# ignaschuemer7/soft-actor-critic

Hardware: AMD Instinct MI355X
Metric: SAC gradient steps/sec + replay-sample GB/s, BipedalWalker batch=256 (higher is better)
Workload: dtype fp32; 1 GPU; c2: BipedalWalker-v3 obs=24 act=4 2x[256, 256] MLPs, buffer=1000000, batch=256, auto-alpha, device sampler, fp32 arithmetic; global_batch=256, parallelism=replicas1, graph_chunk=64

## Files before the change

### soft-actor-critic_amd/csrc/sac_phases.h

```cpp
#pragma once
#include <type_traits>
#include <utility>

#include "sac_device.h"
#include "sac_math.h"

#define SAC_DEV_LAYERS 6

__device__ __forceinline__ __amdgpu_buffer_rsrc_t coh_rsrc(const void* base, uint32_t bytes) {
  return __builtin_amdgcn_make_buffer_rsrc((void*)base, (short)0, (int)bytes, 0x00020000);
}
template <bool COH>
__device__ __forceinline__ void coh_store16(const void* base, uint32_t byte_off, u32x4 v) {
  __builtin_amdgcn_raw_buffer_store_b128(__builtin_bit_cast(__attribute__((ext_vector_type(4))) unsigned, v),
                                         coh_rsrc(base, 0xFFFFFFF0u), (int)byte_off, 0, COH ? 16 : 0);
}
__device__ __forceinline__ float coh_load(const float* p) {
  return __hip_atomic_load((float*)p, __ATOMIC_RELAXED, __HIP_MEMORY_SCOPE_AGENT);
}
template <bool COH>
__device__ __forceinline__ float ldf(const float* p) {
  if constexpr (COH) return coh_load(p);
  return *GPC(float, p);
}
// ... 304 lines not shown
      constexpr int u = decltype(uc)::value;
      f0[u] = coh_frag<T, COH>(rs, o0 + u * FSB);
      f1[u] = coh_frag<T, COH>(rs, o1 + u * FSB);
    });
  }
  F a[NCH][RT];
  static_for<NCH>([&](auto uc) {
    constexpr int u = decltype(uc)::value;
#pragma unroll
    for (int rt = 0; rt < RT; ++rt) a[u][rt] = MM<T>::from_lds(arow + rt * 16 * lda + u * KC);
  });
  f32x4 acc0[RT], acc1[RT];
#pragma unroll
  for (int rt = 0; rt < RT; ++rt) acc0[rt] = acc1[rt] = (f32x4){0.f, 0.f, 0.f, 0.f};
  static_for<NCH>([&](auto uc) {
    constexpr int u = decltype(uc)::value;
#pragma unroll
    for (int rt = 0; rt < RT; ++rt) {
      MM<T>::mma(acc0[rt], a[u][rt], f0[u]);
      MM<T>::mma(acc1[rt], a[u][rt], f1[u]);
    }
  });
  epi(0, nt0 * 16 + c, acc0, true);
  epi(1, nt1 * 16 + c, acc1, true);
}

template <typename T, int ROWS, int HC, typename Epi>
__device__ __forceinline__ void gemm_step(const lf* __restrict__ A, int lda, const GemmW& w, Epi epi,
                                          const Held<T, HC ? HC : 1>* held) {
  constexpr int RT = ROWS / 16;
  constexpr int KC = MM<T>::KC, KL = MM<T>::KL;
  const int lane = threadIdx.x & 63, wave = wave_id();
  const int c = lane & 15, g = lane >> 4;
  const int NT = w.NT, nch = w.cols / KC;
  const lf* arow = A + c * lda + g * KL;
  if (w.NT == 2 * SAC_NW) {
    if (nch == 8) {
      gemm_pair_fixed<T, RT, 8, false, HC>(arow, lda, w, lane, wave, c, epi, held);
      return;
    }
    if (nch == 1) {
      gemm_pair_fixed<T, RT, 1, false, HC>(arow, lda, w, lane, wave, c, epi, held);
      return;
    }
  }
  const __amdgpu_buffer_rsrc_t rs = coh_rsrc(w.p, 0xFFFFFFF0u);
  auto pair = [&](int nt0, bool first) __attribute__((always_inline)) {
    const int nt1 = nt0 + SAC_NW;
    const bool has1 = nt1 < NT;
    const uint32_t o0 = (uint32_t)(packed_lane<T>(nt0, w.tcols, lane) * sizeof(T));
    const uint32_t o1 = (uint32_t)(packed_lane<T>(has1 ? nt1 : nt0, w.tcols, lane) * sizeof(T));
    f32x4 acc0[RT], acc1[RT];
#pragma unroll
    for (int rt = 0; rt < RT; ++rt) acc0[rt] = acc1[rt] = (f32x4){0.f, 0.f, 0.f, 0.f};
    if (HC > 0 && first && held && held->tag == w.p) {
      const int hn = nch < HC ? nch : HC;
      if (hn == HC) {
        mma_batch<T, RT, (HC ? HC : 1)>(arow, lda, 0, has1, held->f0, held->f1, acc0, acc1);
      } else {
        static_for<(HC ? HC : 1)>([&](auto uc) {
          constexpr int u = decltype(uc)::value;
          if (u < hn)
#pragma unroll
            for (int rt = 0; rt < RT; ++rt) {
              const typename MM<T>::Frag a = MM<T>::from_lds(arow + rt * 16 * lda + u * KC);
              MM<T>::mma(acc0[rt], a, held->f0[u]);
              if (has1) MM<T>::mma(acc1[rt], a, held->f1[u]);
            }
        });
      }
      if (hn < nch) mma_pair_from<T, RT, 8>(arow, lda, rs, o0, o1, has1, hn, nch, acc0, acc1);
    } else {
      mma_pair_from<T, RT, 8>(arow, lda, rs, o0, o1, has1, 0, nch, acc0, acc1);
    }
    epi(0, nt0 * 16 + c, acc0, first);
    if (has1) epi(1, nt1 * 16 + c, acc1, first);
  };
  bool first = true;
  for (int nt0 = wave; nt0 < NT; nt0 += 2 * SAC_NW) {
    pair(nt0, first);
    first = false;
  }
}

template <int ROWS>
__device__ __forceinline__ void act_pass_fwd(lf* Y, int ldy, int NT, int act) {
  const int lane = threadIdx.x & 63, wave = wave_id();
  const int c = lane & 15, g = lane >> 4;
#pragma unroll 1
  for (int nt = wave; nt < NT; nt += SAC_NW)
#pragma unroll 1
    for (int e = 0; e < ROWS / 4; ++e) {
      const int r = (e >> 2) * 16 + g * 4 + (e & 3);
      lf* y = Y + r * ldy + nt * 16 + c;
      *y = act_fwd(act, *y);
    }
}
template <int ROWS>
__device__ __forceinline__ void act_pass_bwd(lf* G, int ldg, const lf* P, int ldp, int NT, int K, int act) {
  const int lane = threadIdx.x & 63, wave = wave_id();
  const int c = lane & 15, g = lane >> 4;
#pragma unroll 1
  for (int nt = wave; nt < NT; nt += SAC_NW) {
    const int k = nt * 16 + c;
    if (k >= K) continue;
#pragma unroll 1
    for (int e = 0; e < ROWS / 4; ++e) {
      const int r = (e >> 2) * 16 + g * 4 + (e & 3);
      G[r * ldg + k] = act_bwd(act, P[r * ldp + k], G[r * ldg + k]);
    }
  }
}

template <typename T, int ROWS, int HC = 0>
__device__ __forceinline__ void layer_fwd(const lf* X, int ldx, const AS_C LayerDev& L, const float* bias_, int act, lf* P,
                                          int ldp, lf* Y, int ldy, float* Pg_, int pg_row0,
                                          const Held<T, HC ? HC : 1>* held = nullptr) {
  const AS_G float* bias = GPC(float, bias_);
  AS_G float* Pg = GP(float, Pg_);
  const int lane = threadIdx.x & 63, wave = wave_id();
  const int g = lane >> 4;
  const int N = L.N, Np = L.Np;
  const int n0 = wave * 16 + (lane & 15), n1 = n0 + 16 * SAC_NW;
  const GemmW w = gw_fwd(L);
  const bool hb = HC > 0 && held && held->tag == w.p;
  const float bpre0 = hb ? held->b0 : ldf<false>((const float*)bias + (n0 < N ? n0 : N - 1));
  const float bpre1 = hb ? held->b1 : ldf<false>((const float*)bias + (n1 < N ? n1 : N - 1));
  gemm_step<T, ROWS, HC>(X, ldx, w, [&](int h, int n, const f32x4* acc, bool first) {
    const bool nv = n < N;
    const float bn = first ? (h ? bpre1 : bpre0) : ldf<false>((const float*)bias + (nv ? n : N - 1));
#pragma unroll
    for (int rt = 0; rt < ROWS / 16; ++rt)
#pragma unroll
      for (int i = 0; i < 4; ++i) {
        const int r = rt * 16 + g * 4 + i;
        const float p = nv ? acc[rt][i] + bn : 0.f;
        if (P) P[r * ldp + n] = p;
        Y[r * ldy + n] = act == ACT_RELU ? (p > 0.f ? p : 0.f) : p;
        if (Pg && r >= pg_row0) Pg[(size_t)(r - pg_row0) * Np + n] = p;
      }
  }, held);
  if (act != ACT_RELU && act != ACT_ID) act_pass_fwd<ROWS>(Y, ldy, Np >> 4, act);
}

template <typename T, int ROWS, int HC = 0>
__device__ __forceinline__ void layer_bwd(const lf* G, int ldg, const AS_C LayerDev& L, const lf* Pprev, int ldp,
                                          int act_prev, lf* Gout, int ldo, const Held<T, HC ? HC : 1>* held = nullptr) {
  const int g = (threadIdx.x & 63) >> 4;
  const int K = L.K;
  gemm_step<T, ROWS, HC>(G, ldg, gw_bwd(L), [&](int, int k, const f32x4* acc, bool) {
    const bool kv = k < K;
#pragma unroll
    for (int rt = 0; rt < ROWS / 16; ++rt)
#pragma unroll
      for (int i = 0; i < 4; ++i) {
        const int r = rt * 16 + g * 4 + i;
        float v = kv ? acc[rt][i] : 0.f;
        if (act_prev == ACT_RELU && !(Pprev[r * ldp + k] > 0.f)) v = 0.f;
        Gout[r * ldo + k] = v;
      }
  }, held);
  if (act_prev >= 0 && act_prev != ACT_RELU && act_prev != ACT_ID)
    act_pass_bwd<ROWS>(Gout, ldo, Pprev, ldp, L.Kp >> 4, K, act_prev);
}

template <typename T, int ROWS>
__device__ __forceinline__ void store_T(const lf* __restrict__ src, int lds_ld, int Kp, int K, void* dst_,
                                                 int Bp, int col0, int nvalid, float* dbp_,
                                                 const lf* __restrict__ rowscale = nullptr, int dbp_ld = 0) {
  AS_G T* dst = GP(T, dst_);
  AS_G float* dbp = GP(float, dbp_);
  constexpr int CH = ROWS / 8;
  const int span = (Kp * CH + 63) / 64 * 64;
  for (int i = threadIdx.x; i < span; i += SAC_THREADS) {
    const bool live = i < Kp * CH;
    const int k = i / CH, ch = i % CH;
    T v[8];
    float s = 0.f, xv[8];
#pragma unroll
    for (int q = 0; q < 8; ++q) xv[q] = src[(ch * 8 + q) * lds_ld + (live ? k : 0)];
    if (rowscale) {
      float sc[8];
#pragma unroll
      for (int q = 0; q < 8; ++q) sc[q] = rowscale[ch * 8 + q];
#pragma unroll
      for (int q = 0; q < 8; ++q) xv[q] = sc[q] * xv[q];
    }
#pragma unroll
    for (int q = 0; q < 8; ++q) {
      const int r = ch * 8 + q;
      const float x = (live && r < nvalid && k < K) ? xv[q] : 0.f;
      s += x;
      v[q] = MM<T>::cvt(x);
    }
    if (live) {
      AS_G T* d = dst + (size_t)k * Bp + col0 + ch * 8;
      if constexpr (sizeof(T) == 2) {
        *(AS_G u32x4*)d = *(const u32x4*)v;
      } else {
        *(AS_G u32x4*)d = *(const u32x4*)v;
        *(AS_G u32x4*)(d + 4) = *(const u32x4*)(v + 4);
      }
    }
    if (dbp) {
#pragma unroll
      for (int o = 1; o < CH; o <<= 1) s += __shfl_xor(s, o, 64);
      if (live && ch == 0 && k < K) {
        AS_G float* bp = dbp + (size_t)(col0 / SAC_ROWS) * (dbp_ld ? dbp_ld : K) + k;
        *bp = s;
      }
    }
  }
}

template <typename T, int ROWS, bool HELD = false>
__device__ __forceinline__ void mlp_forward(const AS_C NetDev& net, lf* Xb, lf* Yb, int ld, lf* Pout, lf* Yout, int ldo,
                                            const AS_C int* o_P, const AS_C int* ldp, lf* lds, bool keepP, bool storeXT, int Bp,
                                            int col0, int nvalid, const Held<T, 1>* h0 = nullptr,
                                            const Held<T, 8>* h1 = nullptr) {
  lf* X = Xb;
  lf* Y = Yb;
  for (int l = 0; l < net.L; ++l) {
    const AS_C LayerDev& Ly = net.l[l];
    const bool out = l == net.L - 1;
    if (storeXT) {
      if constexpr (ROWS == SAC_ROWS) store_T<T, ROWS>(X, ld, Ly.Kp, Ly.K, Ly.XT, Bp, col0, nvalid, nullptr);
    }
    const int act = out ? net.out_act : net.hid_act;
    lf* Pl = out ? Pout : (keepP ? lds + o_P[l] : nullptr);
    const int ldpl = out ? ldo : (keepP ? ldp[l] : 0);
    lf* Yl = out ? Yout : Y;
    const int ldyl = out ? ldo : ld;
    if (HELD && l == 0)
      layer_fwd<T, ROWS, 1>(X, ld, Ly, net.P + Ly.b_off, act, Pl, ldpl, Yl, ldyl, nullptr, 0, h0);
    else if (HELD && l == 1)
      layer_fwd<T, ROWS, 8>(X, ld, Ly, net.P + Ly.b_off, act, Pl, ldpl, Yl, ldyl, nullptr, 0, h1);
    else
      layer_fwd<T, ROWS>(X, ld, Ly, net.P + Ly.b_off, act, Pl, ldpl, Yl, ldyl, nullptr, 0);
    __syncthreads();
    lf* t = X;
    X = Y;
    Y = t;
  }
}

template <typename T, int ROWS, bool HELD = false>
__device__ __forceinline__ lf* mlp_backward(const AS_C NetDev& net, const lf* Gout, int ldo, lf* Xb, lf* Yb, int ld,
                                            const AS_C int* o_P, const AS_C int* ldp, lf* lds, bool storeGT, int Bp, int col0,
                                            int nvalid, const Held<T, 1>* h0 = nullptr,
                                            const Held<T, 8>* h1 = nullptr) {
  const int Lh = net.L - 1;
  const AS_C LayerDev& Lo = net.l[Lh];
  if (storeGT) store_T<T, ROWS>(Gout, ldo, Lo.Np, Lo.N, Lo.GT, Bp, col0, nvalid, Lo.dbp);
  layer_bwd<T, ROWS, HELD ? 1 : 0>(Gout, ldo, Lo, lds + o_P[Lh - 1], ldp[Lh - 1], net.hid_act, Yb, ld,
                                   (const Held<T, 1>*)h0);
  __syncthreads();
  lf* G = Yb;
  lf* Gn = Xb;
  for (int l = Lh - 1; l >= 0; --l) {
    const AS_C LayerDev& Ly = net.l[l];
    if (storeGT) store_T<T, ROWS>(G, ld, Ly.Np, Ly.N, Ly.GT, Bp, col0, nvalid, Ly.dbp);
    if (l == 0) break;
    if (HELD && l == Lh - 1)
      layer_bwd<T, ROWS, 8>(G, ld, Ly, lds + o_P[l - 1], ldp[l - 1], net.hid_act, Gn, ld, h1);
    else
      layer_bwd<T, ROWS>(G, ld, Ly, lds + o_P[l - 1], ldp[l - 1], net.hid_act, Gn, ld);
    __syncthreads();
    lf* t = G;
    G = Gn;
    Gn = t;
  }
  __syncthreads();
  return G;
}

template <typename T, int ROWS>
__device__ __forceinline__ void critic_unit_backward(const AS_C EngineDev& E, const AS_C NetDev& net, const lf* Gout, int ldo,
                                                     lf* lds) {
  const int Lh = net.L - 1;
  layer_bwd<T, ROWS>(Gout, ldo, net.l[Lh], lds + E.o_P1[Lh - 1], E.ldp1[Lh - 1], net.hid_act, lds + E.o_P2[Lh - 1],
                     E.ldp2[Lh - 1]);
  __syncthreads();
  for (int l = Lh - 1; l >= 1; --l) {
    layer_bwd<T, ROWS>(lds + E.o_P2[l], E.ldp2[l], net.l[l], lds + E.o_P1[l - 1], E.ldp1[l - 1], net.hid_act,
                       lds + E.o_P2[l - 1], E.ldp2[l - 1]);
    __syncthreads();
  }
}

__device__ __forceinline__ float adam_elem(float& p, float& m, float& v, float g, float w1, float b2, float w2,
                                           float bc2s, float eps, float neg_step) {
  const float mm = m + w1 * (g - m);
  float vv = v * b2;
  vv = vv + (w2 * g) * g;
  const float denom = sqrtf(vv) / bc2s + eps;
  const float pn = p + (neg_step * mm) / denom;
  m = mm;
  v = vv;
  p = pn;
  return pn;
}

#define SAC_UPD_THREADS 1024
#define SAC_UPD_BCH (512 / (int)sizeof(T))
#define SAC_UPD_SLOT_BYTES (64 * 528)
#define SAC_UPD_LDS_FOR(slots) ((slots) * SAC_UPD_SLOT_BYTES + 2 * 32 * 33 * 4 + 32 * 17 * 4 + (slots) * 256 * 4)
#define SAC_UPD_PART_BYTES (4 * 32 * 33 * 4)
__device__ __forceinline__ lf* upd_partials() {
  __shared__ float part[SAC_UPD_PART_BYTES / 4];
  return (lf*)part;
}
template <typename T, int UT, int GS = 1, int MS = 2>
__device__ __forceinline__ void dw_adam_tile(const AS_C EngineDev& E, const TileDesc* tdp_, bool polyak, int par,
                                             int par_x, lf* lds) {
  constexpr int KC = MM<T>::KC, KL = MM<T>::KL;
  constexpr int EPR = 16 / sizeof(T);
  constexpr int EPT = 1024 / UT;
  static_assert(EPR == KL, "a piece is one lane's fragment slice");
  const AS_C TileDesc& td = *(const AS_C TileDesc*)tdp_;
  STAMP(polyak ? 48 : 52);
  const int tid = threadIdx.x;
  const int Bp = td.bp;
  const int lds_row = SAC_UPD_BCH + 16 / (int)sizeof(T);
  AS_L T* stage = (AS_L T*)lds;
  const int nslot = E.upd_slots;
  constexpr int MAXS = MS, PPO = 32 * (SAC_UPD_BCH / EPR) / UT;
  const int ns = nslot < MAXS ? nslot : MAXS;
  const int slot_el = 64 * lds_row;
  lf* accs = lds + (ns * slot_el * (int)sizeof(T) + 15) / 16 * 4;
  lf* tgts = accs + 32 * 33;
  lf* red = tgts + 32 * 33;
  const float neg_step = GPC(float, E.adam_sc)[par * 6 + td.opt * 2];
  const float bc2s = GPC(float, E.adam_sc)[par * 6 + td.opt * 2 + 1];
  static_assert(PPO >= 1 && (32 * (SAC_UPD_BCH / EPR)) % UT == 0, "whole pieces per thread");
  const int rstep = ns * SAC_UPD_BCH;
  u32x4 rg[MAXS][GS + 1][PPO];
  const AS_G float* const seedp = GPC(float, td.seed);
  const bool lseeds = seedp && sizeof(T) == 4 && Bp > rstep;
  AS_L float* seedL = (AS_L float*)(red + 32 * 17);
  f32x4 sreg[MAXS];
  constexpr int SQ = EPR / 4;
  f32x4 sdr[MAXS][PPO][SQ];
  const AS_G T* const gsrc = GPC(T, td.GT);
  const AS_G T* const xsrc = GPC(T, td.XT) + par_x * td.xt_par;
  const long goff = GS > 1 ? td.goff : 0;
  const int ldg = td.ld, ldx = td.ldx;
  auto issue_seeds = [&](int r0, auto slc) __attribute__((always_inline)) {
    constexpr int sl = decltype(slc)::value;
    const int b0 = r0 + sl * SAC_UPD_BCH;
    if (lseeds && sl < ns && b0 < Bp) {
      const int bch = Bp - b0 < SAC_UPD_BCH ? Bp - b0 : SAC_UPD_BCH;
      if (threadIdx.x * 4 < bch) sreg[sl] = *(const AS_G f32x4*)(seedp + b0 + threadIdx.x * 4);
    }
  };
  auto issue = [&](int r0, auto slc, bool seeds = true) {
    constexpr int sl = decltype(slc)::value;
    const int b0 = r0 + sl * SAC_UPD_BCH;
    if (sl < ns && b0 < Bp) {
      const int bch = Bp - b0 < SAC_UPD_BCH ? Bp - b0 : SAC_UPD_BCH;
      const int per_row = bch / EPR;
      if (seeds) issue_seeds(r0, slc);
#pragma unroll
      for (int op = 0; op <= GS; ++op)
#pragma unroll
        for (int pi = 0; pi < PPO; ++pi) {
          const int i = threadIdx.x + pi * UT;
          const int row = i / per_row, pc = i % per_row;
          const AS_G T* src = op < GS ? gsrc + op * goff + (size_t)row * ldg : xsrc + (size_t)row * ldx;
          if (i < 32 * per_row) rg[sl][op][pi] = *(const AS_G u32x4*)(src + b0 + pc * EPR);
          if (op == 0 && seedp && !lseeds && i < 32 * per_row)
#pragma unroll
            for (int q = 0; q < SQ; ++q) sdr[sl][pi][q] = *(const AS_G f32x4*)(seedp + b0 + pc * EPR + 4 * q);
        }
    }
  };
  static_for<MAXS>([&](auto sl) { issue_seeds(0, sl); });
  static_for<MAXS>([&](auto sl) { issue(0, sl, false); });
  auto seeds_to_lds = [&](int r0) __attribute__((always_inline)) {
    if (lseeds)
      static_for<MAXS>([&](auto slc) {
        constexpr int sl = decltype(slc)::value;
        const int b0 = r0 + sl * SAC_UPD_BCH;
        if (sl < ns && b0 < Bp) {
          const int bch = Bp - b0 < SAC_UPD_BCH ? Bp - b0 : SAC_UPD_BCH;
          if (tid * 4 < bch) *(AS_L f32x4*)(seedL + sl * SAC_UPD_BCH + tid * 4) = sreg[sl];
        }
      });
  };
  AS_G float* W = GP(float, td.W);
  AS_G float* Wm = GP(float, td.Wm);
  AS_G float* Wv = GP(float, td.Wv);
  AS_G float* tW = GP(float, td.tW);
  float p[EPT], m[EPT], v[EPT], tp[EPT];
  size_t idx[EPT];
  bool ok[EPT];
#pragma unroll
  for (int e = 0; e < EPT; ++e) {
    const int el = tid + e * UT, en = el >> 5, ek = el & 31;
    const int n = td.n0 + en, k = td.k0 + ek;
    ok[e] = n < td.N && k < td.K;
    idx[e] = ok[e] ? (size_t)n * td.K + k : 0;
    if (td.kpart < 2) {
      p[e] = W[idx[e]];
      m[e] = Wm[idx[e]];
      v[e] = Wv[idx[e]];
      tp[e] = polyak ? tW[idx[e]] : 0.f;
    } else {
      p[e] = m[e] = v[e] = tp[e] = 0.f;
    }
  }
  const bool do_bias = td.k0 == 0 && td.kpart <= 1;
  const bool bias_acc = td.k0 == 0;
  float pb = 0.f, mb = 0.f, vb = 0.f, tbv = 0.f;
  if (do_bias && tid < 32 && td.n0 + tid < td.N) {
    pb = GPC(float, td.b)[td.n0 + tid];
    mb = GPC(float, td.bm)[td.n0 + tid];
    vb = GPC(float, td.bv)[td.n0 + tid];
    if (polyak) tbv = GPC(float, td.tb)[td.n0 + tid];
  }
  constexpr int BPT = (512 + UT - 1) / UT;
  float bsum[BPT];
#pragma unroll
  for (int j = 0; j < BPT; ++j) bsum[j] = 0.f;
  const int lane = tid & 63, wave = wave_id();
  const int c = lane & 15, g = lane >> 4;
  constexpr int KQ = 4, NWV = UT / 64, PPW = 16 / NWV;
  static_assert(UT % 64 == 0 && 16 % NWV == 0, "16 (sub-tile, K-quarter) pairs over whole waves");
  f32x4 acc[PPW];
#pragma unroll
  for (int j = 0; j < PPW; ++j) acc[j] = f32x4{0.f, 0.f, 0.f, 0.f};
  seeds_to_lds(0);
  if (lseeds) __syncthreads();
  auto stage_slot = [&](auto slc, int bch) __attribute__((always_inline)) {
    constexpr int sl = decltype(slc)::value;
    const int per_row = bch / EPR;
#pragma unroll
    for (int op = 0; op < 2; ++op)
#pragma unroll
      for (int pi = 0; pi < PPO; ++pi) {
        const int i = tid + pi * UT;
        const int row = i / per_row + 32 * op, pc = i % per_row;
        u32x4 v = rg[sl][op ? GS : 0][pi];
        if constexpr (sizeof(T) == 4) {
          if constexpr (GS > 1)
            if (op == 0) {
              f32x4 a = __builtin_bit_cast(f32x4, v);
#pragma unroll
              for (int q = 1; q < GS; ++q) a += __builtin_bit_cast(f32x4, rg[sl][q][pi]);
              v = __builtin_bit_cast(u32x4, a);
            }
          if (op == 0 && seedp)
            v = __builtin_bit_cast(u32x4, __builtin_bit_cast(f32x4, v) *
                                              (lseeds ? *(const AS_L f32x4*)(seedL + sl * SAC_UPD_BCH + pc * EPR)
                                                      : sdr[sl][pi][0]));
        } else if (op == 0 && (GS > 1 || seedp)) {
          bf16x8 h = __builtin_bit_cast(bf16x8, v);
          float a[8];
#pragma unroll
          for (int e = 0; e < 8; ++e) a[e] = (float)h[e];
#pragma unroll
          for (int q = 1; q < GS; ++q) {
            const bf16x8 hq = __builtin_bit_cast(bf16x8, rg[sl][q][pi]);
#pragma unroll
            for (int e = 0; e < 8; ++e) a[e] += (float)hq[e];
          }
          if (seedp)
#pragma unroll
            for (int e = 0; e < 8; ++e) a[e] *= sdr[sl][pi][e >> 2][e & 3];
#pragma unroll
          for (int e = 0; e < 8; ++e) h[e] = (bf16)a[e];
          v = __builtin_bit_cast(u32x4, h);
        }
        if (i < 32 * per_row) *(AS_L u32x4*)(stage + sl * slot_el + row * lds_row + pc * EPR) = v;
      }
  };
  constexpr int NIT = SAC_UPD_BCH / KC / KQ;
  constexpr int NBP = SAC_UPD_BCH / (16 * EPR);
  bool single = false;
  if constexpr (UT == SAC_UPD_THREADS) single = Bp <= rstep;
  float gel[EPT];
  if (single) {
    if constexpr (UT == SAC_UPD_THREADS) {
      static_assert(PPW == 1 && BPT == 1, "one (sub-tile, K-quarter) pair per wave");
      typedef typename MM<T>::Frag Frag;
      static_for<MAXS>([&](auto slc) {
        constexpr int sl = decltype(slc)::value;
        const int b0 = sl * SAC_UPD_BCH;
        if (sl < ns && b0 < Bp) stage_slot(slc, Bp - b0 < SAC_UPD_BCH ? Bp - b0 : SAC_UPD_BCH);
      });
      __syncthreads();
      STAMP(polyak ? 51 : 55);
      const int kq = wave >> 2, sn = ((wave & 3) >> 1) * 16, sk = (wave & 1) * 16;
      const int bn = tid >> 4, bs = tid & 15;
      const bool bias_lane = bias_acc && tid < 512;
      auto dw_and_bias = [&](auto fullc) __attribute__((always_inline)) {
        constexpr bool FULL = decltype(fullc)::value;
        Frag fa[MAXS][NIT], fb[MAXS][NIT], bx[MAXS][NBP];
        auto slots = [&](auto&& f) __attribute__((always_inline)) {
          static_for<MAXS>([&](auto slc) {
            constexpr int sl = decltype(slc)::value;
            const int b0 = sl * SAC_UPD_BCH;
            if (sl < ns && b0 < Bp)
              f(slc, FULL || Bp - b0 >= SAC_UPD_BCH ? SAC_UPD_BCH : Bp - b0);
          });
        };
        slots([&](auto slc, int bch) {
          constexpr int sl = decltype(slc)::value;
          const AS_L T* arow = stage + sl * slot_el + (sn + c) * lds_row + g * KL;
          const AS_L T* brow = stage + sl * slot_el + (32 + sk + c) * lds_row + g * KL;
#pragma unroll
          for (int it = 0; it < NIT; ++it) {
            const int ch = kq + it * KQ;
            if (FULL || ch < bch / KC) {
              fa[sl][it] = *(const AS_L Frag*)(arow + ch * KC);
              fb[sl][it] = *(const AS_L Frag*)(brow + ch * KC);
            }
          }
        });
        if (bias_lane)
          slots([&](auto slc, int bch) {
            constexpr int sl = decltype(slc)::value;
#pragma unroll
            for (int it = 0; it < NBP; ++it) {
              const int bc = (bs + it * 16) * EPR;
              if (FULL || bc < bch) bx[sl][it] = *(const AS_L Frag*)(stage + sl * slot_el + bn * lds_row + bc);
            }
          });
        slots([&](auto slc, int bch) {
          constexpr int sl = decltype(slc)::value;
#pragma unroll
          for (int it = 0; it < NIT; ++it)
            if (FULL || kq + it * KQ < bch / KC) MM<T>::mma(acc[0], fa[sl][it], fb[sl][it]);
        });
        if (bias_lane)
          slots([&](auto slc, int bch) {
            constexpr int sl = decltype(slc)::value;
#pragma unroll
            for (int it = 0; it < NBP; ++it)
              if (FULL || (bs + it * 16) * EPR < bch) {
                const Frag x = bx[sl][it];
                if constexpr (sizeof(T) == 4) {
                  bsum[0] += (x[0] + x[1]) + (x[2] + x[3]);
                } else {
                  float s = 0.f;
#pragma unroll
                  for (int e = 0; e < 8; ++e) s += (float)x[e];
                  bsum[0] += s;
                }
              }
          });
      };
      if (Bp % SAC_UPD_BCH == 0)
        dw_and_bias(std::true_type{});
      else
        dw_and_bias(std::false_type{});
      STAMP(polyak ? 49 : 53);
      lf* part = upd_partials();
#pragma unroll
      for (int i = 0; i < 4; ++i) part[kq * (32 * 33) + (sn + g * 4 + i) * 33 + sk + c] = acc[0][i];
      if (bias_lane) red[bn * 17 + bs] = bsum[0];
      __syncthreads();
#pragma unroll
      for (int e = 0; e < EPT; ++e) {
        const int el = tid + e * UT, o = (el >> 5) * 33 + (el & 31);
        float sum = part[o];
#pragma unroll
        for (int q = 1; q < KQ; ++q) sum += part[q * (32 * 33) + o];
        gel[e] = sum;
      }
    }
  } else {
    for (int r0 = 0; r0 < Bp; r0 += rstep) {
      static_for<MAXS>([&](auto slc) {
        constexpr int sl = decltype(slc)::value;
        const int b0 = r0 + sl * SAC_UPD_BCH;
        if (sl < ns && b0 < Bp) {
          const int bch = Bp - b0 < SAC_UPD_BCH ? Bp - b0 : SAC_UPD_BCH;
          stage_slot(slc, bch);
          issue(r0 + rstep, slc);
          __syncthreads();
          if (r0 == 0 && sl == 0) STAMP(polyak ? 51 : 55);
          if (bias_acc) {
#pragma unroll
            for (int j = 0; j < BPT; ++j) {
              const int t = tid + j * UT, bn = t >> 4, bs = t & 15;
              if (t < 512)
                for (int c = bs * EPR; c < bch; c += 16 * EPR) {
                  const AS_L T* q = stage + sl * slot_el + bn * lds_row + c;
                  if constexpr (sizeof(T) == 4) {
                    const f32x4 x = *(const AS_L f32x4*)q;
                    bsum[j] += (x[0] + x[1]) + (x[2] + x[3]);
                  } else {
                    const bf16x8 x = *(const AS_L bf16x8*)q;
                    float s = 0.f;
#pragma unroll
                    for (int e = 0; e < 8; ++e) s += (float)x[e];
                    bsum[j] += s;
                  }
                }
            }
          }
#pragma unroll
          for (int j = 0; j < PPW; ++j) {
            const int pr = wave + j * NWV, kq = pr >> 2;
            const int ns = ((pr & 3) >> 1) * 16, ks = (pr & 1) * 16;
            const AS_L T* arow = stage + sl * slot_el + (ns + c) * lds_row + g * KL;
            const AS_L T* brow = stage + sl * slot_el + (32 + ks + c) * lds_row + g * KL;
            for (int ch = kq; ch < bch / KC; ch += KQ) {
              typename MM<T>::Frag a, b;
              if constexpr (sizeof(T) == 2) {
                a = *(const AS_L bf16x8*)(arow + ch * KC);
                b = *(const AS_L bf16x8*)(brow + ch * KC);
              } else {
                a = *(const AS_L f32x4*)(arow + ch * KC);
                b = *(const AS_L f32x4*)(brow + ch * KC);
              }
              MM<T>::mma(acc[j], a, b);
            }
          }
        }
      });
      seeds_to_lds(r0 + rstep);
      __syncthreads();
    }
    STAMP(polyak ? 49 : 53);
    {
#pragma unroll
      for (int j = 0; j < PPW; ++j) {
        const int pr = wave + j * NWV;
        const int ns = ((pr & 3) >> 1) * 16, ks = (pr & 1) * 16;
        lf* part = (lf*)stage + (pr >> 2) * (32 * 33);
#pragma unroll
        for (int i = 0; i < 4; ++i) part[(ns + g * 4 + i) * 33 + ks + c] = acc[j][i];
      }
    }
    __syncthreads();
    for (int el = tid; el < 1024; el += UT) {
      const int o = (el >> 5) * 33 + (el & 31);
      const lf* part = (const lf*)stage;
      float sum = part[o];
#pragma unroll
      for (int q = 1; q < KQ; ++q) sum += part[q * (32 * 33) + o];
      accs[o] = sum;
    }
#pragma unroll
    for (int j = 0; j < BPT; ++j) {
      const int t = tid + j * UT;
      if (bias_acc && t < 512) red[(t >> 4) * 17 + (t & 15)] = bsum[j];
    }
    __syncthreads();
  }
  constexpr int MAXP = UT == 512 ? 7 : 3;
  float gbx[MAXP];
#pragma unroll
  for (int q = 0; q < MAXP; ++q) gbx[q] = 0.f;
  if (td.kpart) {
    const uint32_t ep = *GPC(uint32_t, E.sync) + 1u;
    if (td.kpart >= 2) {
      AS_G uint64_t* mine = GP(uint64_t, td.part) + (size_t)(td.kpart - 2) * SAC_PART_STRIDE;
#pragma unroll
      for (int e = 0; e < EPT; ++e) {
        const int el = tid + e * UT;
        const float dw = single ? gel[e] : accs[(el >> 5) * 33 + (el & 31)];
        const uint64_t x = (uint64_t)__float_as_uint(dw) | ((uint64_t)ep << 32);
        __hip_atomic_store((uint64_t*)(mine + el), x, __ATOMIC_RELAXED, __HIP_MEMORY_SCOPE_AGENT);
      }
      if (bias_acc && tid < 32) {
        float gb = 0.f;
        for (int q = 0; q < 16; ++q) gb += red[tid * 17 + q];
        const uint64_t x = (uint64_t)__float_as_uint(gb) | ((uint64_t)ep << 32);
        __hip_atomic_store((uint64_t*)(mine + 1024 + tid), x, __ATOMIC_RELAXED, __HIP_MEMORY_SCOPE_AGENT);
      }
      return;
    }
    constexpr int EL = 1024 / UT;
    static_assert(EL * UT == 1024 && EL <= 4, "granules per thread");
    const int np = td.nparts - 1;
    const bool pb_here = do_bias && tid < 32;
    float v[MAXP][EL];
    for (int it = 0;; ++it) {
      bool all = true;
#pragma unroll
      for (int q = 0; q < MAXP; ++q)
        if (q < np) {
#pragma unroll
          for (int j = 0; j < EL; ++j) {
            const uint64_t x = __hip_atomic_load(td.part + (size_t)q * SAC_PART_STRIDE + tid + j * UT,
                                                 __ATOMIC_RELAXED, __HIP_MEMORY_SCOPE_AGENT);
            all = all && (uint32_t)(x >> 32) == ep;
            v[q][j] = __uint_as_float((uint32_t)x);
          }
          if (pb_here) {
            const uint64_t x = __hip_atomic_load(td.part + (size_t)q * SAC_PART_STRIDE + 1024 + tid,
                                                 __ATOMIC_RELAXED, __HIP_MEMORY_SCOPE_AGENT);
            all = all && (uint32_t)(x >> 32) == ep;
            gbx[q] = __uint_as_float((uint32_t)x);
          }
        }
      if (all) break;
      if (it > E.spin_limit) {
        __hip_atomic_store((uint32_t*)GP(uint32_t, E.sync) + 1 , 1u, __ATOMIC_RELAXED,
                           __HIP_MEMORY_SCOPE_AGENT);
        break;
      }
      __builtin_amdgcn_s_sleep(1);
    }
#pragma unroll
    for (int j = 0; j < EL; ++j) {
      const int el = tid + j * UT, o = (el >> 5) * 33 + (el & 31);
      float sum = single ? gel[j] : accs[o];
#pragma unroll
      for (int q = 0; q < MAXP; ++q)
        if (q < np) sum += v[q][j];
      if (single)
        gel[j] = sum;
      else
        accs[o] = sum;
    }
    if (!single) __syncthreads();
  }
  STAMP(polyak ? 50 : 54);
  const float w1 = (float)(1.0 - (double)E.beta1), b2 = E.beta2, w2 = (float)(1.0 - (double)E.beta2);
  const float eps = E.adam_eps, tau = E.tau, omt = (float)(1.0 - (double)E.tau);
  float pn[EPT], tn[EPT];
#pragma unroll
  for (int e = 0; e < EPT; ++e) {
    const int el = tid + e * UT;
    pn[e] = 0.f;
    tn[e] = 0.f;
    if (ok[e]) {
      const float dw = single ? gel[e] : accs[(el >> 5) * 33 + (el & 31)];
      pn[e] = adam_elem(p[e], m[e], v[e], dw, w1, b2, w2, bc2s, eps, neg_step);
      W[idx[e]] = p[e];
      Wm[idx[e]] = m[e];
      Wv[idx[e]] = v[e];
      if (polyak) {
        tn[e] = tau * pn[e] + omt * tp[e];
        tW[idx[e]] = tn[e];
      }
    }
  }
  if (!single) __syncthreads();
#pragma unroll
  for (int e = 0; e < EPT; ++e) {
    const int el = tid + e * UT;
    accs[(el >> 5) * 33 + (el & 31)] = pn[e];
    if (polyak) tgts[(el >> 5) * 33 + (el & 31)] = tn[e];
  }
  if (do_bias && tid < 32 && td.n0 + tid < td.N) {
    float gb = 0.f;
    for (int q = 0; q < 16; ++q) gb += red[tid * 17 + q];
    if (td.kpart) {
#pragma unroll
      for (int q = 0; q < MAXP; ++q)
        if (q < td.nparts - 1) gb += gbx[q];
    }
    const float pbn = adam_elem(pb, mb, vb, gb, w1, b2, w2, bc2s, eps, neg_step);
    GP(float, td.b)[td.n0 + tid] = pb;
    GP(float, td.bm)[td.n0 + tid] = mb;
    GP(float, td.bv)[td.n0 + tid] = vb;
    if (polyak) GP(float, td.tb)[td.n0 + tid] = tau * pbn + omt * tbv;
  }
  __syncthreads();
  constexpr int PPR = 32 / EPR;
  for (int mat = 0; mat < (polyak ? 3 : 2); ++mat) {
    const void* base = mat == 0 ? td.Wc : mat == 1 ? td.WTc : td.tWc;
    for (int i = tid; i < 32 * PPR; i += UT) {
      const int row = i / PPR, pc = i % PPR;
      T vv[EPR];
      size_t off;
      if (mat == 1) {
#pragma unroll
        for (int j = 0; j < EPR; ++j) vv[j] = MM<T>::cvt(accs[(pc * EPR + j) * 33 + row]);
        off = packed_off<T>(td.k0 + row, td.n0 + pc * EPR, td.Np);
      } else {
        const lf* srcm = mat == 0 ? accs : tgts;
#pragma unroll
        for (int j = 0; j < EPR; ++j) vv[j] = MM<T>::cvt(srcm[row * 33 + pc * EPR + j]);
        off = packed_off<T>(td.n0 + row, td.k0 + pc * EPR, td.Kp);
      }
      coh_store16<false>(base, (uint32_t)(off * sizeof(T)), *(const u32x4*)vv);
    }
  }
}

template <typename T, int UT, int MS = 2>
__device__ __forceinline__ void dw_adam_tile_any(const AS_C EngineDev& E, const TileDesc* tdp_, bool polyak, int par,
                                                 int par_x, lf* lds) {
  if constexpr (UT != 512) {
    const int gs = ((const AS_C TileDesc*)tdp_)->gsum;
    if constexpr (sizeof(T) == 4)
      if (gs == 4) return dw_adam_tile<T, UT, 4, MS>(E, tdp_, polyak, par, par_x, lds);
    if (gs == 2) return dw_adam_tile<T, UT, 2, MS>(E, tdp_, polyak, par, par_x, lds);
  }
  dw_adam_tile<T, UT, 1, MS>(E, tdp_, polyak, par, par_x, lds);
}

__device__ __forceinline__ void alpha_and_losses(const AS_C EngineDev& E, int par, lf* red) {
  const int tid = threadIdx.x, NT = blockDim.x, B = E.B;
  const float H = E.target_entropy;
  AS_G double* st = GP(double, E.alpha_state);
  const double st0 = st[0];
  const float la32 = (float)st0;
  const float mB = -1.0f / (float)B;
  const AS_G float* lp = GPC(float, E.lp_st) + par * E.Br;
  const AS_G float* lossp = GPC(float, E.lossp) + par * E.nrt * 4;
  float sg = 0.f, sl = 0.f, l0 = 0.f, l1 = 0.f, l2 = 0.f;
  for (int b = tid; b < B; b += NT) {
    const float term = lp[b] + H;
    sg += mB * term;
    sl += la32 * term;
  }
  for (int rt = tid; rt < E.nrt; rt += NT) {
    l0 += lossp[rt * 4 + 0];
    l1 += lossp[rt * 4 + 1];
    l2 += lossp[rt * 4 + 2];
  }
  red[0 * NT + tid] = sg;
  red[1 * NT + tid] = sl;
  red[2 * NT + tid] = l0;
  red[3 * NT + tid] = l1;
  red[4 * NT + tid] = l2;
  __syncthreads();
  for (int s = NT / 2; s > 0; s >>= 1) {
    if (tid < s)
      for (int j = 0; j < 5; ++j) red[j * NT + tid] += red[j * NT + tid + s];
    __syncthreads();
  }
  if (tid == 0) {
    AS_G float* stats = GP(float, E.stats);
    stats[0] = red[2 * NT] / (float)B;
    stats[1] = red[3 * NT] / (float)B;
    stats[2] = red[4 * NT] / (float)B;
    stats[3] = E.auto_entropy ? -(red[1 * NT] / (float)B) : __builtin_nanf("");
    if (E.auto_entropy && E.alpha_update) {
      const double gr = (double)red[0];
      const double b1 = (double)E.beta1, b2 = (double)E.beta2;
      const double st2 = st[2], st3 = st[3];
      const double m = st2 + (1.0 - b1) * (gr - st2);
      const double v = st3 * b2 + (1.0 - b2) * gr * gr;
      const double bc1 = GPC(double, E.alpha_sc)[par * 2];
      const double bc2 = GPC(double, E.alpha_sc)[par * 2 + 1];
      const double denom = sqrt(v) / sqrt(bc2) + (double)E.adam_eps;
      const double la = st0 + (-(E.alpha_lr / bc1)) * m / denom;
      double* sd = (double*)E.alpha_state;
      __hip_atomic_store(sd + 0, la, __ATOMIC_RELAXED, __HIP_MEMORY_SCOPE_AGENT);
      __hip_atomic_store(sd + 1, exp(la), __ATOMIC_RELAXED, __HIP_MEMORY_SCOPE_AGENT);
      __hip_atomic_store(sd + 2, m, __ATOMIC_RELAXED, __HIP_MEMORY_SCOPE_AGENT);
      __hip_atomic_store(sd + 3, v, __ATOMIC_RELAXED, __HIP_MEMORY_SCOPE_AGENT);
    }
  }
}

enum HandKind { HK_PI = 0, HK_T1 = 1, HK_T2 = 2, HK_C1 = 3, HK_C2 = 4, HK_COUNT = 5 };
enum SyncWord { SYNC_EPOCH = 0, SYNC_TIMEOUT = 1, SYNC_STAGED = 4, SYNC_CDONE = 64, SYNC_FLAGS = 128 };
#define SAC_HAND_STRIDE 576

__device__ __forceinline__ AS_G uint32_t* hand_flag(const AS_C EngineDev& E, int kind, int rbi) {
  return GP(uint32_t, E.sync) + SYNC_FLAGS + (kind * E.nrt + rbi) * 16;
}
__device__ __forceinline__ AS_G float* hand_data(const AS_C EngineDev& E, int kind, int rbi) {
  return GP(float, E.hand) + (size_t)(kind * E.nrt + rbi) * SAC_HAND_STRIDE;
}
__device__ __forceinline__ void st_sc1(AS_G float* p, float v) {
  __hip_atomic_store((float*)p, v, __ATOMIC_RELAXED, __HIP_MEMORY_SCOPE_AGENT);
}
__device__ __forceinline__ float ld_sc1(const AS_G float* p) {
  return __hip_atomic_load((float*)p, __ATOMIC_RELAXED, __HIP_MEMORY_SCOPE_AGENT);
}
__device__ __forceinline__ void hand_publish(const AS_C EngineDev& E, int kind, int rbi, uint32_t ep) {
  asm volatile("s_waitcnt vmcnt(0)" ::: "memory");
  __syncthreads();
  if (threadIdx.x == 0) __hip_atomic_store((uint32_t*)hand_flag(E, kind, rbi), ep, __ATOMIC_RELAXED,
                                           __HIP_MEMORY_SCOPE_AGENT);
}
__device__ __forceinline__ void hand_wait(const AS_C EngineDev& E, int kind, int rbi, uint32_t ep) {
  if (threadIdx.x == 0) {
    uint32_t* f = (uint32_t*)hand_flag(E, kind, rbi);
    for (int it = 0; __hip_atomic_load(f, __ATOMIC_RELAXED, __HIP_MEMORY_SCOPE_AGENT) != ep; ++it) {
      if (it > E.spin_limit) {
        __hip_atomic_store((uint32_t*)GP(uint32_t, E.sync) + 1, 1u, __ATOMIC_RELAXED, __HIP_MEMORY_SCOPE_AGENT);
        break;
      }
      __builtin_amdgcn_s_sleep(2);
    }
  }
  __syncthreads();
}

__device__ __forceinline__ void hand_wait2(const AS_C EngineDev& E, int k1, int k2, int rbi, uint32_t ep) {
  if (threadIdx.x == 0) {
    uint32_t* f1 = (uint32_t*)hand_flag(E, k1, rbi);
    uint32_t* f2 = (uint32_t*)hand_flag(E, k2, rbi);
    for (int it = 0;; ++it) {
      const uint32_t a = __hip_atomic_load(f1, __ATOMIC_RELAXED, __HIP_MEMORY_SCOPE_AGENT);
      const uint32_t b = __hip_atomic_load(f2, __ATOMIC_RELAXED, __HIP_MEMORY_SCOPE_AGENT);
      if (a == ep && b == ep) break;
      if (it > E.spin_limit) {
        __hip_atomic_store((uint32_t*)GP(uint32_t, E.sync) + 1, 1u, __ATOMIC_RELAXED, __HIP_MEMORY_SCOPE_AGENT);
        break;
      }
      __builtin_amdgcn_s_sleep(2);
    }
  }
  __syncthreads();
}

enum GranKind { G_Q1T = 0, G_Q2T = 1, G_LP = 2, G_C1 = 3, G_C2 = 4, G_PI = 5, G_COUNT = 6 };
__device__ __forceinline__ AS_G uint64_t* gran_at(const AS_C EngineDev& E, int kind, int rbi) {
  return GP(uint64_t, E.gran) + (size_t)(kind * E.nrt + rbi) * E.gstride;
}
__device__ __forceinline__ void gran_put(AS_G uint64_t* g, float v, uint32_t ep) {
  const uint64_t x = (uint64_t)__float_as_uint(v) | ((uint64_t)ep << 32);
  __hip_atomic_store((uint64_t*)g, x, __ATOMIC_RELAXED, __HIP_MEMORY_SCOPE_AGENT);
}
__device__ __forceinline__ float gran_get(const AS_C EngineDev& E, const AS_G uint64_t* g, uint32_t ep) {
  uint64_t x = 0;
  for (int it = 0;; ++it) {
    x = __hip_atomic_load((uint64_t*)g, __ATOMIC_RELAXED, __HIP_MEMORY_SCOPE_AGENT);
    if ((uint32_t)(x >> 32) == ep) break;
    if (it > E.spin_limit) {
      __hip_atomic_store((uint32_t*)GP(uint32_t, E.sync) + SYNC_TIMEOUT, 1u, __ATOMIC_RELAXED,
                         __HIP_MEMORY_SCOPE_AGENT);
      break;
    }
    __builtin_amdgcn_s_sleep(1);
  }
  return __uint_as_float((uint32_t)x);
}

#define SAC_POLL_SLEEP 4
template <int N>
__device__ __forceinline__ bool gran_ok(const uint64_t (&x)[N], uint32_t ep) {
  bool all = true;
#pragma unroll
  for (int i = 0; i < N; ++i) all = all && (uint32_t)(x[i] >> 32) == ep;
  return all;
}
template <int N>
__device__ __forceinline__ void gran_issue(const AS_G uint64_t* const (&g)[N], uint64_t (&x)[N]) {
#pragma unroll
  for (int i = 0; i < N; ++i) x[i] = __hip_atomic_load((uint64_t*)g[i], __ATOMIC_RELAXED, __HIP_MEMORY_SCOPE_AGENT);
}
template <int N>
__device__ __forceinline__ void gran_getn1(const AS_C EngineDev& E, const AS_G uint64_t* const (&g)[N], uint32_t ep,
                                           float (&out)[N]) {
  uint64_t x[N];
  for (int it = 0;; ++it) {
#pragma unroll
    for (int i = 0; i < N; ++i) x[i] = __hip_atomic_load((uint64_t*)g[i], __ATOMIC_RELAXED, __HIP_MEMORY_SCOPE_AGENT);
    bool all = true;
#pragma unroll
    for (int i = 0; i < N; ++i) all = all && (uint32_t)(x[i] >> 32) == ep;
    if (all) break;
    if (it > E.spin_limit) {
      __hip_atomic_store((uint32_t*)GP(uint32_t, E.sync) + SYNC_TIMEOUT, 1u, __ATOMIC_RELAXED,
                         __HIP_MEMORY_SCOPE_AGENT);
      break;
    }
    __builtin_amdgcn_s_sleep(1);
  }
#pragma unroll
  for (int i = 0; i < N; ++i) out[i] = __uint_as_float((uint32_t)x[i]);
}
template <int N>
__device__ __forceinline__ void gran_getn(const AS_C EngineDev& E, const AS_G uint64_t* const (&g)[N], uint32_t ep,
                                          float (&out)[N]) {
  uint64_t x[N], y[N];
  gran_issue<N>(g, x);
  __builtin_amdgcn_s_sleep(SAC_POLL_SLEEP);
  gran_issue<N>(g, y);
  for (int it = 0;; it += 2) {
    if (gran_ok<N>(x, ep)) {
#pragma unroll
      for (int i = 0; i < N; ++i) out[i] = __uint_as_float((uint32_t)x[i]);
      return;
    }
    gran_issue<N>(g, x);
    if (gran_ok<N>(y, ep)) {
#pragma unroll
      for (int i = 0; i < N; ++i) out[i] = __uint_as_float((uint32_t)y[i]);
      return;
    }
    if (it > E.spin_limit) {
      __hip_atomic_store((uint32_t*)GP(uint32_t, E.sync) + SYNC_TIMEOUT, 1u, __ATOMIC_RELAXED,
                         __HIP_MEMORY_SCOPE_AGENT);
#pragma unroll
      for (int i = 0; i < N; ++i) out[i] = __uint_as_float((uint32_t)y[i]);
      return;
    }
    gran_issue<N>(g, y);
  }
}

__device__ __forceinline__ void tile_slots(const AS_C EngineDev& E, const sac_replay& rb, uint64_t step,
                                           int64_t rb_size, int64_t rb_pos, int r0, const AS_G int32_t* inj_idx,
                                           AS_L int64_t* slotB) {
  const int tid = threadIdx.x;
  if (tid < SAC_ROWS) {
    int64_t slot = -1;
    const int b = r0 + tid;
    if (b < E.B) {
      int64_t li;
      if (inj_idx) {
        li = inj_idx[b];
      } else {
        const Feistel f = feistel_make(E.seed, step, rb_size);
        li = feistel_sample(f, b, rb_size);
      }
      slot = rb_size < rb.capacity ? li : (rb_pos + li) % rb.capacity;
    }
    slotB[tid] = slot;
  }
}

template <typename Dst>
__device__ __forceinline__ void gather_rows(const sac_replay& rb, const AS_L int64_t* slotB, int O, int A, Dst s,
                                            Dst s2, Dst a, Dst r, Dst d) {
  constexpr int R = SAC_ROWS;
  const AS_G float* obs = GPC(float, rb.obs);
  const AS_G float* nobs = GPC(float, rb.next_obs);
  const AS_G float* ract = GPC(float, rb.act);
  const AS_G float* rrew = GPC(float, rb.rew);
  const AS_G float* rdone = GPC(float, rb.done);
  const RowStrides rs = row_strides(rb.row_stride, O, A);
  const int nI = R * (O > A ? O : A);
  for (int i = threadIdx.x; i < nI; i += SAC_THREADS) {
    const int io = i < R * O ? i : R * O - 1, ia = i < R * A ? i : R * A - 1, ir = i < R ? i : R - 1;
    const int64_t so = slotB[io / O], sa = slotB[ia / A], sr = slotB[ir];
    const int64_t po = (so < 0 ? 0 : so) * rs.obs + io % O, pa = (sa < 0 ? 0 : sa) * rs.act + ia % A,
                  pr = (sr < 0 ? 0 : sr) * rs.one;
    const float vo = obs[po], vn = nobs[po], va = ract[pa], vr = rrew[pr], vd = rdone[pr];
    if (i < R * O) {
      s[i] = so >= 0 ? vo : 0.f;
      s2[i] = so >= 0 ? vn : 0.f;
    }
    if (i < R * A) a[i] = sa >= 0 ? va : 0.f;
    if (i < R) {
      r[i] = sr >= 0 ? vr : 0.f;
      d[i] = sr >= 0 ? vd : 0.f;
    }
  }
}

__device__ __forceinline__ size_t stage_rec(const AS_C EngineDev& E, uint64_t step, int rbi) {
  return ((size_t)(step & 1) * E.nrt + rbi) * E.stg_stride;
}
__device__ __forceinline__ void stage_next_batch(const AS_C EngineDev& E, const sac_replay& rb, int rbi, lf* lds,
                                                 uint64_t cur_step) {
  constexpr int R = SAC_ROWS;
  const uint64_t step = cur_step + 1;
  const int64_t rb_size = GPC(int64_t, rb.state)[0], rb_pos = GPC(int64_t, rb.state)[1];
  AS_G float* rec = GP(float, E.stg) + stage_rec(E, step, rbi);
  AS_G uint64_t* hdr = (AS_G uint64_t*)rec;
  if (rb_size < E.B) {
    if (threadIdx.x == 0) hdr[0] = ~0ull;
    return;
  }
  AS_L int64_t* slotB = (AS_L int64_t*)lds;
  tile_slots(E, rb, step, rb_size, rb_pos, rbi * R, nullptr, slotB);
  __syncthreads();
  const int O = E.O, A = E.A;
  AS_G float* p = rec + 16;
  gather_rows<AS_G float*>(rb, slotB, O, A, p, p + R * O, p + 2 * R * O, p + 2 * R * O + R * A,
                           p + 2 * R * O + R * A + R);
  if (threadIdx.x == 0) {
    hdr[0] = step;
    hdr[1] = (uint64_t)rb_size;
    hdr[2] = (uint64_t)rb_pos;
    hdr[3] = (uint64_t)(uintptr_t)rb.obs;
    hdr[4] = (uint64_t)GPC(int64_t, rb.state)[2];
  }
}

template <typename T, bool ROLES>
__device__ __forceinline__ void target_critic_body(const EngineDev* __restrict__ Ep, const sac_replay& rb,
                                                   const int32_t* __restrict__ inj_idx_,
                                                   const float* __restrict__ inj_eps_) {
  PREFETCH_ARG(Ep);
  const AS_C EngineDev& E = *(const AS_C EngineDev*)Ep;
  extern __shared__ float lds_raw[];
  lf* lds = (lf*)lds_raw;
  constexpr int R = SAC_ROWS;
  const int tid = threadIdx.x;
  const int bid = blockIdx.x;
  int rbi, role;
  if (ROLES) {
    rbi = bid % E.nrt;
    role = bid / E.nrt;
  } else {
    if (blockIdx.x % E.xs) return;
    rbi = blockIdx.x / E.xs;
    role = -1;
  }
  const bool do_pi = !ROLES || role == 0 || role == 5;
  STAMP(0);
  CLK_STAMP(40);
  const int B = E.B, Bp = E.Bp, O = E.O, A = E.A, ld = E.ld, ldo = E.ldo;
// ... 713 lines not shown
```

Before: 23000 gradient steps/s.

## Specialize single-round Adam tiles and coalesce fp32 master weight stores via LDS

Makes the single-round path a compile-time template parameter, chosen by the dispatcher from the batch-per-tile size, so the two paths are compiled separately instead of branching at runtime. For aligned full 32x32 tiles in the single path, Adam moment and parameter writes are staged in LDS and written back as 16-byte coherent buffer stores per row, replacing scattered scalar global stores. Packed weight copies use coherent stores in the single path. A double-buffered polling variant for partial sums is added but disabled by a macro; the change costs more instantiations, code size and extra LDS staging passes.

```diff
diff --git a/soft-actor-critic_amd/csrc/sac_phases.h b/soft-actor-critic_amd/csrc/sac_phases.h
--- a/soft-actor-critic_amd/csrc/sac_phases.h
+++ b/soft-actor-critic_amd/csrc/sac_phases.h
@@ -630,6 +630,7 @@
 }
 
 #define SAC_UPD_THREADS 1024
+#define SAC_UPD_POLL2 0
 #define SAC_UPD_BCH (512 / (int)sizeof(T))
 #define SAC_UPD_SLOT_BYTES (64 * 528)
 #define SAC_UPD_LDS_FOR(slots) ((slots) * SAC_UPD_SLOT_BYTES + 2 * 32 * 33 * 4 + 32 * 17 * 4 + (slots) * 256 * 4)
@@ -638,7 +639,7 @@
   __shared__ float part[SAC_UPD_PART_BYTES / 4];
   return (lf*)part;
 }
-template <typename T, int UT, int GS = 1, int MS = 2>
+template <typename T, int UT, int GS, int MS, bool ONE>
 __device__ __forceinline__ void dw_adam_tile(const AS_C EngineDev& E, const TileDesc* tdp_, bool polyak, int par,
                                              int par_x, lf* lds) {
   constexpr int KC = MM<T>::KC, KL = MM<T>::KL;
@@ -804,8 +805,8 @@
   };
   constexpr int NIT = SAC_UPD_BCH / KC / KQ;
   constexpr int NBP = SAC_UPD_BCH / (16 * EPR);
-  bool single = false;
-  if constexpr (UT == SAC_UPD_THREADS) single = Bp <= rstep;
+  static_assert(!ONE || UT == SAC_UPD_THREADS, "single-round tiles: the 1024-thread kernels");
+  constexpr bool single = ONE;
   float gel[EPT];
   if (single) {
     if constexpr (UT == SAC_UPD_THREADS) {
@@ -1006,6 +1007,63 @@
     const int np = td.nparts - 1;
     const bool pb_here = do_bias && tid < 32;
     float v[MAXP][EL];
+#if SAC_UPD_POLL2
+    uint64_t xa[MAXP][EL + 1], xb[MAXP][EL + 1];
+    auto poll = [&](uint64_t(&x)[MAXP][EL + 1]) __attribute__((always_inline)) {
+#pragma unroll
+      for (int q = 0; q < MAXP; ++q)
+        if (q < np) {
+#pragma unroll
+          for (int j = 0; j < EL; ++j)
+            x[q][j] = __hip_atomic_load(td.part + (size_t)q * SAC_PART_STRIDE + tid + j * UT, __ATOMIC_RELAXED,
+                                        __HIP_MEMORY_SCOPE_AGENT);
+          if (pb_here)
+            x[q][EL] = __hip_atomic_load(td.part + (size_t)q * SAC_PART_STRIDE + 1024 + tid, __ATOMIC_RELAXED,
+                                         __HIP_MEMORY_SCOPE_AGENT);
+        }
+    };
+    auto landed = [&](const uint64_t(&x)[MAXP][EL + 1]) __attribute__((always_inline)) {
+      bool all = true;
+#pragma unroll
+      for (int q = 0; q < MAXP; ++q)
+        if (q < np) {
+#pragma unroll
+          for (int j = 0; j < EL; ++j) all = all && (uint32_t)(x[q][j] >> 32) == ep;
+          if (pb_here) all = all && (uint32_t)(x[q][EL] >> 32) == ep;
+        }
+      return all;
+    };
+    auto take = [&](const uint64_t(&x)[MAXP][EL + 1]) __attribute__((always_inline)) {
+#pragma unroll
+      for (int q = 0; q < MAXP; ++q)
+        if (q < np) {
+#pragma unroll
+          for (int j = 0; j < EL; ++j) v[q][j] = __uint_as_float((uint32_t)x[q][j]);
+          if (pb_here) gbx[q] = __uint_as_float((uint32_t)x[q][EL]);
+        }
+    };
+    poll(xa);
+    __builtin_amdgcn_s_sleep(4);
+    poll(xb);
+    for (int it = 0;; it += 2) {
+      if (landed(xa)) {
+        take(xa);
+        break;
+      }
+      poll(xa);
+      if (landed(xb)) {
+        take(xb);
+        break;
+      }
+      if (it > E.spin_limit) {
+        __hip_atomic_store((uint32_t*)GP(uint32_t, E.sync) + 1 , 1u, __ATOMIC_RELAXED,
+                           __HIP_MEMORY_SCOPE_AGENT);
+        take(xb);
+        break;
+      }
+      poll(xb);
+    }
+#else
     for (int it = 0;; ++it) {
       bool all = true;
 #pragma unroll
@@ -1033,6 +1091,7 @@
       }
       __builtin_amdgcn_s_sleep(1);
     }
+#endif
 #pragma unroll
     for (int j = 0; j < EL; ++j) {
       const int el = tid + j * UT, o = (el >> 5) * 33 + (el & 31);
@@ -1051,6 +1110,10 @@
   const float w1 = (float)(1.0 - (double)E.beta1), b2 = E.beta2, w2 = (float)(1.0 - (double)E.beta2);
   const float eps = E.adam_eps, tau = E.tau, omt = (float)(1.0 - (double)E.tau);
   float pn[EPT], tn[EPT];
+  const bool rows = single && td.n0 + 32 <= td.N && td.k0 + 32 <= td.K && td.K % 32 == 0 &&
+                    (((uintptr_t)td.W | (uintptr_t)td.Wm | (uintptr_t)td.Wv | (polyak ? (uintptr_t)td.tW : 0)) & 127) == 0;
+  lf* const mrow = (lf*)stage;
+  lf* const vrow = mrow + 32 * 33;
 #pragma unroll
   for (int e = 0; e < EPT; ++e) {
     const int el = tid + e * UT;
@@ -1059,12 +1122,15 @@
     if (ok[e]) {
       const float dw = single ? gel[e] : accs[(el >> 5) * 33 + (el & 31)];
       pn[e] = adam_elem(p[e], m[e], v[e], dw, w1, b2, w2, bc2s, eps, neg_step);
-      W[idx[e]] = p[e];
-      Wm[idx[e]] = m[e];
-      Wv[idx[e]] = v[e];
-      if (polyak) {
-        tn[e] = tau * pn[e] + omt * tp[e];
-        tW[idx[e]] = tn[e];
+      if (polyak) tn[e] = tau * pn[e] + omt * tp[e];
+      if (rows) {
+        mrow[(el >> 5) * 33 + (el & 31)] = m[e];
+        vrow[(el >> 5) * 33 + (el & 31)] = v[e];
+      } else {
+        W[idx[e]] = p[e];
+        Wm[idx[e]] = m[e];
+        Wv[idx[e]] = v[e];
+        if (polyak) tW[idx[e]] = tn[e];
       }
     }
   }
@@ -1090,6 +1156,19 @@
     if (polyak) GP(float, td.tb)[td.n0 + tid] = tau * pbn + omt * tbv;
   }
   __syncthreads();
+  if (rows)
+    for (int mat = 0; mat < (polyak ? 4 : 3); ++mat) {
+      const float* base = mat == 0 ? td.W : mat == 1 ? td.Wm : mat == 2 ? td.Wv : td.tW;
+      const lf* srcm = mat == 0 ? accs : mat == 1 ? mrow : mat == 2 ? vrow : tgts;
+      for (int i = tid; i < 32 * 8; i += UT) {
+        const int row = i >> 3, pc = i & 7;
+        float vv[4];
+#pragma unroll
+        for (int j = 0; j < 4; ++j) vv[j] = srcm[row * 33 + pc * 4 + j];
+        coh_store16<true>(base, (uint32_t)(((size_t)(td.n0 + row) * td.K + td.k0 + pc * 4) * sizeof(float)),
+                          *(const u32x4*)vv);
+      }
+    }
   constexpr int PPR = 32 / EPR;
   for (int mat = 0; mat < (polyak ? 3 : 2); ++mat) {
     const void* base = mat == 0 ? td.Wc : mat == 1 ? td.WTc : td.tWc;
@@ -1107,7 +1186,10 @@
         for (int j = 0; j < EPR; ++j) vv[j] = MM<T>::cvt(srcm[row * 33 + pc * EPR + j]);
         off = packed_off<T>(td.n0 + row, td.k0 + pc * EPR, td.Kp);
       }
-      coh_store16<false>(base, (uint32_t)(off * sizeof(T)), *(const u32x4*)vv);
+      if (single)
+        coh_store16<true>(base, (uint32_t)(off * sizeof(T)), *(const u32x4*)vv);
+      else
+        coh_store16<false>(base, (uint32_t)(off * sizeof(T)), *(const u32x4*)vv);
     }
   }
 }
@@ -1115,13 +1197,22 @@
 template <typename T, int UT, int MS = 2>
 __device__ __forceinline__ void dw_adam_tile_any(const AS_C EngineDev& E, const TileDesc* tdp_, bool polyak, int par,
                                                  int par_x, lf* lds) {
+  auto run = [&](auto gsc) __attribute__((always_inline)) {
+    constexpr int GS = decltype(gsc)::value;
+    if constexpr (UT == SAC_UPD_THREADS) {
+      const int ns = E.upd_slots < MS ? E.upd_slots : MS;
+      if (((const AS_C TileDesc*)tdp_)->bp <= ns * SAC_UPD_BCH)
+        return dw_adam_tile<T, UT, GS, MS, true>(E, tdp_, polyak, par, par_x, lds);
+    }
+    dw_adam_tile<T, UT, GS, MS, false>(E, tdp_, polyak, par, par_x, lds);
+  };
   if constexpr (UT != 512) {
     const int gs = ((const AS_C TileDesc*)tdp_)->gsum;
     if constexpr (sizeof(T) == 4)
-      if (gs == 4) return dw_adam_tile<T, UT, 4, MS>(E, tdp_, polyak, par, par_x, lds);
-    if (gs == 2) return dw_adam_tile<T, UT, 2, MS>(E, tdp_, polyak, par, par_x, lds);
-  }
-  dw_adam_tile<T, UT, 1, MS>(E, tdp_, polyak, par, par_x, lds);
+      if (gs == 4) return run(std::integral_constant<int, 4>{});
+    if (gs == 2) return run(std::integral_constant<int, 2>{});
+  }
+  run(std::integral_constant<int, 1>{});
 }
 
 __device__ __forceinline__ void alpha_and_losses(const AS_C EngineDev& E, int par, lf* red) {
```

After: 23230 gradient steps/s, median of 6. No clear change (+1.0%).
